# ErlerPhilipp/points2surf

Hardware: NVIDIA H100
Metric: SDF queries/sec at grid_res=256 (higher is better)
Workload: dtype f16 operands / f32 accumulate (wgmma); hi/lo split f16 (fp32-level) for FC tails and guard-band recompute

## Files before the change

points2surf_b200/csrc/net_tc.cu:

```cuda
#include "model.cuh"
#include "tc_ptx.cuh"

namespace p2s {

using namespace ptx;

namespace {

constexpr int kTile = 64;
constexpr int kWG = 2;
constexpr int kThreads = 128 * kWG;
constexpr uint32_t kAct2Bytes = kTile * 128 * 2;
template <bool PRECISE>
struct Cfg {
    static constexpr int kChunks = PRECISE ? 1 : 4;
    static constexpr int kSplit = 8 / kChunks;
    static constexpr uint32_t kChunkBytes = PRECISE ? 65536u : 32768u;
    static constexpr uint32_t kW3Bytes = kChunks * kChunkBytes;
    static constexpr uint32_t kMidScale = PRECISE ? 2u : 1u;
    static constexpr uint32_t kMidBytes = (8192u + 8192u + 16384u) * kMidScale;
    static constexpr uint32_t kPerqBytes = PRECISE ? 16384u : 8192u;
    static constexpr uint32_t kOffMid = kW3Bytes;
    static constexpr uint32_t kWgPerq = kAct2Bytes * kMidScale;
    static constexpr uint32_t kWgWq = kWgPerq + kPerqBytes;
    static constexpr uint32_t kWgBytes = kWgWq + 192 * 4;
    static constexpr uint32_t kOffWg = kOffMid + kMidBytes;
    static constexpr uint32_t kOffBias = kOffWg + kWG * kWgBytes;
    static constexpr uint32_t kSmemBytes = kOffBias + 320 * 4;
};
static_assert(Cfg<false>::kSmemBytes <= 232448 && Cfg<true>::kSmemBytes <= 232448, "shared memory budget");

struct Seg {
    const float* ptr;
    int n;
    int tiles;
    int center;
};

struct PassParams {
    Seg seg[2];
    const float* query;
    const float* R;
    int tiles_per_query;
    int B;
    const float* W0;
    const float* b0;
    int num_mid;
    int mid_N[3];
    const uint8_t* mid_img[3];
    const float* mid_bias[3];
    int perq_layer;
    const uint8_t* perq_img;
    const uint8_t* w3_img;
    float* out;
};

__device__ __forceinline__ uint32_t pack_relu(float a, float b) {
    uint32_t r;
    asm("cvt.rn.relu.satfinite.f16x2.f32 %0, %1, %2;" : "=r"(r) : "f"(b), "f"(a));
    return r;
}
__device__ __forceinline__ void pack_relu_split(float a, float b, uint32_t& hi, uint32_t& lo) {
    hi = pack_relu(a, b);
    const float2 hf = __half22float2(*reinterpret_cast<const __half2*>(&hi));
    lo = pack_half2(fmaxf(a, 0.f) - hf.x, fmaxf(b, 0.f) - hf.y);
}
template <bool PRECISE>
__device__ __forceinline__ void pack_act(float a, float b, uint32_t& hi, uint32_t& lo) {
    if (PRECISE) pack_relu_split(a, b, hi, lo);
    else hi = pack_relu(a, b);
}

template <bool PRECISE, int R>
__device__ __forceinline__ void mid_mma(float (&d)[R], const uint32_t (&a)[4], const uint32_t (&al)[4], uint64_t w, uint64_t w_lo, uint32_t acc) {
    if (R == 32) {
        auto& d32 = reinterpret_cast<float (&)[32]>(d);
        if (PRECISE) { wgmma_rs_n64(d32, al, w, acc); wgmma_rs_n64(d32, a, w_lo, 1); wgmma_rs_n64(d32, a, w, 1); }
        else wgmma_rs_n64(d32, a, w, acc);
    } else {
        auto& d64 = reinterpret_cast<float (&)[64]>(d);
        if (PRECISE) { wgmma_rs_n128(d64, al, w, acc); wgmma_rs_n128(d64, a, w_lo, 1); wgmma_rs_n128(d64, a, w, 1); }
        else wgmma_rs_n128(d64, a, w, acc);
    }
}

template <bool PRECISE>
__global__ void __launch_bounds__(kThreads, 1) pointnet_pass_kernel(const PassParams p) {
    using C = Cfg<PRECISE>;
    constexpr int kL = PRECISE ? 4 : 1;
    extern __shared__ __align__(1024) uint8_t smem[];
    float* s_bias = reinterpret_cast<float*>(smem + C::kOffBias);
    const int tid = threadIdx.x, wg = tid >> 7, t = tid & 127, lane = tid & 31, q4 = lane & 3;
    const int r0 = (t >> 5) * 16 + (lane >> 2);
    const int part = blockIdx.x % C::kSplit;
    const int stream = blockIdx.x / C::kSplit, nstreams = gridDim.x / C::kSplit;
    const int nq = (p.B > stream) ? (p.B - stream + nstreams - 1) / nstreams : 0;
    const int tpq = p.tiles_per_query;
    uint32_t mid_off[3] = {0, 0, 0};
    {
        uint32_t o = 0;
        for (int l = 0; l < p.num_mid; ++l) { mid_off[l] = o; o += (uint32_t)p.mid_N[l] * 128u * C::kMidScale; }
    }

    if (nq > 0) {
        const uint4* src = reinterpret_cast<const uint4*>(p.w3_img + (size_t)part * C::kW3Bytes);
        uint4* dst = reinterpret_cast<uint4*>(smem);
        for (uint32_t i = tid; i < C::kW3Bytes / 16; i += kThreads) dst[i] = src[i];
        for (int l = 0; l < p.num_mid; ++l) {
            if (l == p.perq_layer) continue;
            const uint4* s = reinterpret_cast<const uint4*>(p.mid_img[l]);
            uint4* d = reinterpret_cast<uint4*>(smem + C::kOffMid + mid_off[l]);
            for (uint32_t i = tid; i < (uint32_t)p.mid_N[l] * 8u * C::kMidScale; i += kThreads) d[i] = s[i];
        }
    }
    {
        int off = 0;
        for (int l = 0; l < p.num_mid; ++l) {
            for (int i = tid; i < p.mid_N[l]; i += kThreads) s_bias[off + i] = p.mid_bias[l][i];
            off += p.mid_N[l];
        }
        for (int i = tid; i < 64; i += kThreads) s_bias[256 + i] = p.b0[i];
    }
    fence_proxy_async_smem();
    __syncthreads();

    uint8_t* wsm = smem + C::kOffWg + wg * C::kWgBytes;
    uint8_t* act2 = wsm;
    uint8_t* perq = wsm + C::kWgPerq;
    float* wq = reinterpret_cast<float*>(wsm + C::kWgWq);
    const float* s_b0 = s_bias + 256;
    const uint32_t bar_id = 1 + (uint32_t)wg;
    auto wg_sync = [&]() { asm volatile("bar.sync %0, 128;" ::"r"(bar_id) : "memory"); };
    const uint64_t dsc_act2 = make_smem_desc(smem_u32(act2), 128, 2048);
    const uint64_t dsc_w3 = make_smem_desc(smem_u32(smem), 128, 2048);
    uint64_t dsc_mid[3], dsc_mid_lo[3];
    for (int l = 0; l < 3; ++l) {
        const bool pq = l == p.perq_layer;
        dsc_mid[l] = make_smem_desc(pq ? smem_u32(perq) : smem_u32(smem + C::kOffMid) + mid_off[l], 128, 1024);
        dsc_mid_lo[l] = dsc_mid[l] + (uint64_t)((pq ? 8192u : (uint32_t)p.mid_N[l] * 128u) >> 4);
    }

    for (int qi = wg; qi < nq; qi += kWG) {
        const size_t q = (size_t)stream + (size_t)qi * nstreams;
        wg_sync();
        if (t < 64) {
            const float w0 = p.W0[t * 3 + 0], w1 = p.W0[t * 3 + 1], w2 = p.W0[t * 3 + 2];
            float r[9] = {1.f, 0.f, 0.f, 0.f, 1.f, 0.f, 0.f, 0.f, 1.f};
            if (p.R) {
#pragma unroll
                for (int i = 0; i < 9; ++i) r[i] = p.R[q * 9 + i];
            }
            wq[0 * 64 + t] = w0 * r[0] + w1 * r[3] + w2 * r[6];
            wq[1 * 64 + t] = w0 * r[1] + w1 * r[4] + w2 * r[7];
            wq[2 * 64 + t] = w0 * r[2] + w1 * r[5] + w2 * r[8];
        }
        if (p.perq_layer >= 0) {
            const uint4* s = reinterpret_cast<const uint4*>(p.perq_img + q * C::kPerqBytes);
            uint4* d = reinterpret_cast<uint4*>(perq);
            for (uint32_t i = t; i < C::kPerqBytes / 16; i += 128) d[i] = s[i];
            fence_proxy_async_smem();
        }
        wg_sync();
        float rmax[4 * C::kChunks];
#pragma unroll
        for (int i = 0; i < 4 * C::kChunks; ++i) rmax[i] = -INFINITY;
        for (int tq = 0; tq < tpq; ++tq) {
            const int sgi = tq < p.seg[0].tiles ? 0 : 1;
            const Seg& sg = p.seg[sgi];
            float cx = 0.f, cy = 0.f, cz = 0.f;
            if (sg.center) { cx = p.query[q * 3 + 0]; cy = p.query[q * 3 + 1]; cz = p.query[q * 3 + 2]; }
            float px[2], py[2], pz[2];
#pragma unroll
            for (int h = 0; h < 2; ++h) {
                int local = (tq - (sgi ? p.seg[0].tiles : 0)) * kTile + r0 + 8 * h;
                if (local >= sg.n) local = 0;
                const float* src = sg.ptr + (q * sg.n + local) * 3;
                px[h] = src[0] - cx; py[h] = src[1] - cy; pz[h] = src[2] - cz;
            }
            uint32_t a[4][4], al[4][kL];
#pragma unroll
            for (int kk = 0; kk < 4; ++kk) {
#pragma unroll
                for (int hc = 0; hc < 2; ++hc) {
                    const int ch = kk * 16 + hc * 8 + 2 * q4;
                    const float2 wx = *reinterpret_cast<const float2*>(wq + 0 * 64 + ch);
                    const float2 wy = *reinterpret_cast<const float2*>(wq + 1 * 64 + ch);
                    const float2 wz = *reinterpret_cast<const float2*>(wq + 2 * 64 + ch);
                    const float2 bb = *reinterpret_cast<const float2*>(s_b0 + ch);
#pragma unroll
                    for (int h = 0; h < 2; ++h) {
                        const float v0 = fmaf(wx.x, px[h], fmaf(wy.x, py[h], fmaf(wz.x, pz[h], bb.x)));
                        const float v1 = fmaf(wx.y, px[h], fmaf(wy.y, py[h], fmaf(wz.y, pz[h], bb.y)));
                        pack_act<PRECISE>(v0, v1, a[kk][hc * 2 + h], al[kk][PRECISE ? hc * 2 + h : 0]);
                    }
                }
            }
            int boff = 0;
            for (int l = 0; l < p.num_mid; ++l) {
                const float* bl = s_bias + boff;
                const uint64_t w = dsc_mid[l], w_lo = dsc_mid_lo[l];
                if (l < p.num_mid - 1) {
                    float d[32];
#pragma unroll
                    for (int i = 0; i < 32; ++i) d[i] = 0.f;
                    wgmma_fence();
#pragma unroll
                    for (int ks = 0; ks < 4; ++ks)
                        mid_mma<PRECISE>(d, a[ks], reinterpret_cast<const uint32_t (&)[4]>(al[PRECISE ? ks : 0]), w + (uint64_t)(ks * 16), w_lo + (uint64_t)(ks * 16), ks > 0);
                    wgmma_commit();
                    wgmma_wait<0>();
                    fence_regs(d);
#pragma unroll
                    for (int j = 0; j < 8; ++j) {
                        const float2 bb = *reinterpret_cast<const float2*>(bl + 8 * j + 2 * q4);
                        pack_act<PRECISE>(d[4 * j] + bb.x, d[4 * j + 1] + bb.y, a[j >> 1][(j & 1) * 2], al[j >> 1][PRECISE ? (j & 1) * 2 : 0]);
                        pack_act<PRECISE>(d[4 * j + 2] + bb.x, d[4 * j + 3] + bb.y, a[j >> 1][(j & 1) * 2 + 1], al[j >> 1][PRECISE ? (j & 1) * 2 + 1 : 0]);
                    }
                } else {
                    float d[64];
#pragma unroll
                    for (int i = 0; i < 64; ++i) d[i] = 0.f;
                    wgmma_fence();
#pragma unroll
                    for (int ks = 0; ks < 4; ++ks)
                        mid_mma<PRECISE>(d, a[ks], reinterpret_cast<const uint32_t (&)[4]>(al[PRECISE ? ks : 0]), w + (uint64_t)(ks * 16), w_lo + (uint64_t)(ks * 16), ks > 0);
                    wgmma_commit();
                    wgmma_wait<0>();
                    fence_regs(d);
                    wg_sync();
#pragma unroll
                    for (int j = 0; j < 16; ++j) {
                        const int k = 8 * j + 2 * q4;
                        const float2 bb = *reinterpret_cast<const float2*>(bl + k);
#pragma unroll
                        for (int h = 0; h < 2; ++h) {
                            const int pt = r0 + 8 * h;
                            const uint32_t off = (uint32_t)(pt >> 3) * 2048u + (uint32_t)j * 128u + (uint32_t)(pt & 7) * 16u + (uint32_t)q4 * 4u;
                            uint32_t hi, lo = 0;
                            pack_act<PRECISE>(d[4 * j + 2 * h] + bb.x, d[4 * j + 2 * h + 1] + bb.y, hi, lo);
                            *reinterpret_cast<uint32_t*>(act2 + off) = hi;
                            if (PRECISE) *reinterpret_cast<uint32_t*>(act2 + kAct2Bytes + off) = lo;
                        }
                    }
                    fence_proxy_async_smem();
                    wg_sync();
                }
                boff += p.mid_N[l];
            }
#pragma unroll
            for (int c = 0; c < C::kChunks; ++c) {
                float d0[32], d1[32];
#pragma unroll
                for (int i = 0; i < 32; ++i) { d0[i] = 0.f; d1[i] = 0.f; }
                const uint64_t wa = dsc_w3 + (uint64_t)((uint32_t)c * (C::kChunkBytes >> 4)), wb = wa + (uint64_t)(16384u >> 4);
                wgmma_fence();
#pragma unroll
                for (int ks = 0; ks < 8; ++ks) {
                    const uint64_t x = dsc_act2 + (uint64_t)(ks * 16), o = (uint64_t)(ks * 16);
                    if (PRECISE) {
                        const uint64_t x_lo = x + (uint64_t)(kAct2Bytes >> 4), lo = (uint64_t)(32768u >> 4);
                        wgmma_ss_n64(d0, wa + lo + o, x, ks > 0); wgmma_ss_n64(d0, wa + o, x_lo, 1); wgmma_ss_n64(d0, wa + o, x, 1);
                        wgmma_ss_n64(d1, wb + lo + o, x, ks > 0); wgmma_ss_n64(d1, wb + o, x_lo, 1); wgmma_ss_n64(d1, wb + o, x, 1);
                    } else {
                        wgmma_ss_n64(d0, wa + o, x, ks > 0);
                        wgmma_ss_n64(d1, wb + o, x, ks > 0);
                    }
                }
                wgmma_commit();
                wgmma_wait<0>();
                fence_regs(d0);
                fence_regs(d1);
#pragma unroll
                for (int j = 0; j < 8; ++j) {
                    rmax[4 * c + 0] = fmaxf(rmax[4 * c + 0], fmaxf(d0[4 * j], d0[4 * j + 1]));
                    rmax[4 * c + 1] = fmaxf(rmax[4 * c + 1], fmaxf(d0[4 * j + 2], d0[4 * j + 3]));
                    rmax[4 * c + 2] = fmaxf(rmax[4 * c + 2], fmaxf(d1[4 * j], d1[4 * j + 1]));
                    rmax[4 * c + 3] = fmaxf(rmax[4 * c + 3], fmaxf(d1[4 * j + 2], d1[4 * j + 3]));
                }
            }
        }
#pragma unroll
        for (int i = 0; i < 4 * C::kChunks; ++i) {
            rmax[i] = fmaxf(rmax[i], __shfl_xor_sync(0xffffffffu, rmax[i], 1));
            rmax[i] = fmaxf(rmax[i], __shfl_xor_sync(0xffffffffu, rmax[i], 2));
        }
        if (q4 == 0) {
#pragma unroll
            for (int i = 0; i < 4 * C::kChunks; ++i)
                p.out[q * 1024 + (size_t)((part * C::kChunks + (i >> 2)) * 128 + ((i >> 1) & 1) * 64 + r0 + (i & 1) * 8)] = rmax[i];
        }
    }
}

__global__ void pack_kmajor_kernel(const float* __restrict__ W, int rows, int K, int row0, uint32_t sbo, uint8_t* __restrict__ img, int lo) {
    int e = blockIdx.x * blockDim.x + threadIdx.x;
    if (e >= rows * K) return;
    int r = e / K, k = e % K;
    uint32_t off = (uint32_t)(r >> 3) * sbo + (uint32_t)(k >> 3) * 128u + (uint32_t)(r & 7) * 16u + (uint32_t)(k & 7) * 2u;
    const float w = W[(size_t)(row0 + r) * K + k];
    const __half h = __float2half_rn(w);
    *reinterpret_cast<__half*>(img + off) = lo ? __float2half_rn(w - __half2float(h)) : h;
}

__global__ void pack_perq_kernel(const float* __restrict__ W, int64_t B, uint8_t* __restrict__ img) {
    int64_t e = (int64_t)blockIdx.x * blockDim.x + threadIdx.x;
    if (e >= B * 4096) return;
    int64_t b = e >> 12;
    int r = (int)((e >> 6) & 63), k = (int)(e & 63);
    uint32_t off = (uint32_t)(r >> 3) * 1024u + (uint32_t)(k >> 3) * 128u + (uint32_t)(r & 7) * 16u + (uint32_t)(k & 7) * 2u;
    *reinterpret_cast<__half*>(img + b * 8192 + off) = __float2half_rn(W[e]);
}

__global__ void __launch_bounds__(256) fold_w1_kernel(const float* __restrict__ W1, const float* __restrict__ T, int64_t B, uint8_t* __restrict__ img) {
    __shared__ float sW[64][65];
    __shared__ __align__(16) float sT[64][68];
    const int64_t b = blockIdx.x;
    const int tid = threadIdx.x;
    for (int e = tid; e < 4096; e += 256) {
        const int r = e >> 6, c = e & 63;
        sW[r][c] = W1[e];
        sT[r][c] = T[b * 4096 + e] + (r == c ? 1.0f : 0.0f);
    }
    __syncthreads();
    const int o = tid >> 2, i0 = (tid & 3) * 16;
    float acc[16];
#pragma unroll
    for (int i = 0; i < 16; ++i) acc[i] = 0.f;
    for (int j = 0; j < 64; ++j) {
        const float w = sW[o][j];
#pragma unroll
        for (int i4 = 0; i4 < 4; ++i4) {
            const float4 t4 = *reinterpret_cast<const float4*>(&sT[j][i0 + 4 * i4]);
            acc[4 * i4 + 0] = fmaf(w, t4.x, acc[4 * i4 + 0]);
            acc[4 * i4 + 1] = fmaf(w, t4.y, acc[4 * i4 + 1]);
            acc[4 * i4 + 2] = fmaf(w, t4.z, acc[4 * i4 + 2]);
            acc[4 * i4 + 3] = fmaf(w, t4.w, acc[4 * i4 + 3]);
        }
    }
    uint8_t* dst = img + b * 8192 + (uint32_t)(o >> 3) * 1024u + (uint32_t)(o & 7) * 16u;
#pragma unroll
    for (int h = 0; h < 2; ++h) {
        uint32_t v[4];
#pragma unroll
        for (int e = 0; e < 4; ++e) v[e] = pack_half2(acc[h * 8 + 2 * e], acc[h * 8 + 2 * e + 1]);
        *reinterpret_cast<uint4*>(dst + (uint32_t)(i0 / 8 + h) * 128u) = make_uint4(v[0], v[1], v[2], v[3]);
    }
}

__global__ void fold_fc3_kernel(const float* __restrict__ W1, const float* __restrict__ Wfc3, const float* __restrict__ bfc3,
                                float* __restrict__ G, float* __restrict__ g0) {
    const int oi = blockIdx.x;
    const int o = oi >> 6, i = oi & 63;
    const int k = threadIdx.x;
    float acc = 0.f;
    for (int j = 0; j < 64; ++j) acc = fmaf(W1[o * 64 + j], Wfc3[(size_t)(j * 64 + i) * 256 + k], acc);
    G[(size_t)oi * 256 + k] = acc;
    if (k == 0) {
        float b = W1[o * 64 + i];
        for (int j = 0; j < 64; ++j) b = fmaf(W1[o * 64 + j], bfc3[j * 64 + i], b);
        g0[oi] = b;
    }
}

__global__ void transpose64_kernel(const float* __restrict__ in, float* __restrict__ out, int64_t B) {
    int64_t e = (int64_t)blockIdx.x * blockDim.x + threadIdx.x;
    if (e >= B * 4096) return;
    int64_t b = e >> 12;
    int i = (int)((e >> 6) & 63), j = (int)(e & 63);
    out[e] = in[b * 4096 + j * 64 + i];
}

__global__ void guard_flag_kernel(const float* __restrict__ logits, int64_t B, float band, int32_t* __restrict__ list, int* __restrict__ count, int64_t base, int64_t cap) {
    int64_t i = (int64_t)blockIdx.x * blockDim.x + threadIdx.x;
    if (i >= B) return;
    if (fabsf(logits[i * 2 + 1]) < band) {
        int slot = atomicAdd(count, 1);
        if (slot < cap) list[slot] = (int32_t)(base + i);
    }
}
__global__ void guard_gather_kernel(const float* __restrict__ src, const int32_t* __restrict__ list, int n, int row_floats, float* __restrict__ dst) {
    int64_t e = (int64_t)blockIdx.x * blockDim.x + threadIdx.x;
    if (e >= (int64_t)n * row_floats) return;
    int i = (int)(e / row_floats), j = (int)(e % row_floats);
    dst[e] = src[(int64_t)list[i] * row_floats + j];
}
__global__ void guard_scatter_kernel(const float* __restrict__ src, const int32_t* __restrict__ list, int n, float* __restrict__ logits) {
    int i = blockIdx.x * blockDim.x + threadIdx.x;
    if (i >= n) return;
    logits[(int64_t)list[i] * 2 + 0] = src[i * 2 + 0];
    logits[(int64_t)list[i] * 2 + 1] = src[i * 2 + 1];
}

}

struct TcStack {
    uint8_t* w3_img = nullptr;
    uint8_t* mid_img[3] = {nullptr, nullptr, nullptr};
    uint8_t* w3_img_p = nullptr;
    uint8_t* mid_img_p[3] = {nullptr, nullptr, nullptr};
    const float* mid_bias[3] = {nullptr, nullptr, nullptr};
    int mid_N[3] = {0, 0, 0};
    int num_mid = 0;
    const float* W0 = nullptr;
    const float* b0 = nullptr;
    const float* b3 = nullptr;
};

struct TcFc {
    const Layer* L = nullptr;
    const uint8_t* img = nullptr;
};
struct TcStnFc { TcFc fc1, fc2, fc3; };

struct TcWeights {
    TcStack qstn;
    TcStack stn[2], fin[2];
    TcStnFc qstn_fc, stn_fc[2];
    TcFc head_fc1[2], head_fc2, head_fc3;
    const uint8_t* fold_img[2] = {nullptr, nullptr};
    const float* fold_bias[2] = {nullptr, nullptr};
    bool fc_on_tc = true;
    std::vector<void*> allocs;
    int sm_count = 132;
    bool prof_on = false;
    std::vector<std::pair<cudaEvent_t, cudaEvent_t>> prof_events;
    double prof_flops = 0.0;
    ~TcWeights() {
        for (void* a : allocs) cudaFree(a);
        for (auto& e : prof_events) { cudaEventDestroy(e.first); cudaEventDestroy(e.second); }
    }
};

namespace {

uint8_t* tc_alloc(TcWeights& t, size_t bytes) {
    void* p = nullptr;
    P2S_CUDA(cudaMalloc(&p, bytes));
    P2S_CUDA(cudaMemset(p, 0, bytes));
    t.allocs.push_back(p);
    return (uint8_t*)p;
}

uint8_t* pack_layer(TcWeights& t, const Layer& L, uint32_t sbo, bool split = false) {
    const size_t one = (size_t)L.cout * L.cin * 2;
    uint8_t* img = tc_alloc(t, one * (split ? 2 : 1));
    P2S_LAUNCH(pack_kmajor_kernel, (unsigned)cdiv((int64_t)L.cout * L.cin, 256), 256, 0, 0, L.W, L.cout, L.cin, 0, sbo, img, 0);
    if (split) P2S_LAUNCH(pack_kmajor_kernel, (unsigned)cdiv((int64_t)L.cout * L.cin, 256), 256, 0, 0, L.W, L.cout, L.cin, 0, sbo, img + one, 1);
    return img;
}

uint8_t* pack_w3(TcWeights& t, const Layer& L, bool split = false) {
    P2S_CHECK(L.cout == 1024 && L.cin == 128, "big layer must be 128 -> 1024");
    const size_t chunk = split ? 65536 : 32768;
    uint8_t* img = tc_alloc(t, 8 * chunk);
    for (int c = 0; c < 8; ++c) {
        P2S_LAUNCH(pack_kmajor_kernel, (unsigned)cdiv(128 * 128, 256), 256, 0, 0, L.W, 128, 128, c * 128, 2048u, img + (size_t)c * chunk, 0);
        if (split) P2S_LAUNCH(pack_kmajor_kernel, (unsigned)cdiv(128 * 128, 256), 256, 0, 0, L.W, 128, 128, c * 128, 2048u, img + (size_t)c * chunk + 32768, 1);
    }
    return img;
}

void launch_pass(Model& m, const TcStack& s, const Seg& s0, const Seg& s1, const float* query, const float* R,
                 int64_t B, int perq_layer, const uint8_t* perq_img, float* out, cudaStream_t st, bool precise) {
    PassParams p{};
    p.seg[0] = s0; p.seg[1] = s1;
    p.query = query; p.R = R;
    p.tiles_per_query = s0.tiles + s1.tiles;
    p.B = (int)B;
    p.W0 = s.W0; p.b0 = s.b0;
    p.num_mid = s.num_mid;
    for (int l = 0; l < 3; ++l) { p.mid_N[l] = s.mid_N[l]; p.mid_img[l] = precise ? s.mid_img_p[l] : s.mid_img[l]; p.mid_bias[l] = s.mid_bias[l]; }
    p.perq_layer = perq_layer;
    p.perq_img = perq_img;
    p.w3_img = precise ? s.w3_img_p : s.w3_img;
    p.out = out;
    for (int l = 0; l < s.num_mid; ++l)
        P2S_CHECK(s.mid_N[l] == (l == s.num_mid - 1 ? 128 : 64), "pass kernel: mid layers must be 64 -> 64 ... -> 128");
    TcWeights& t = *m.tc;
    const int split = precise ? Cfg<true>::kSplit : Cfg<false>::kSplit;
    int streams = t.sm_count / split;
    if ((int64_t)streams > B) streams = (int)B;
    const int grid = streams * split;
    cudaEvent_t e0 = nullptr, e1 = nullptr;
    const bool prof = t.prof_on && !precise;
    if (prof) {
        P2S_CUDA(cudaEventCreate(&e0)); P2S_CUDA(cudaEventCreate(&e1));
        P2S_CUDA(cudaEventRecord(e0, st));
    }
    if (precise) P2S_LAUNCH(pointnet_pass_kernel<true>, grid, kThreads, Cfg<true>::kSmemBytes, st, p);
    else P2S_LAUNCH(pointnet_pass_kernel<false>, grid, kThreads, Cfg<false>::kSmemBytes, st, p);
    if (prof) {
        P2S_CUDA(cudaEventRecord(e1, st));
        t.prof_events.emplace_back(e0, e1);
        double mac_pt = 3.0 * 64 + 128.0 * 1024;
        int prev = 64;
        for (int l = 0; l < s.num_mid; ++l) { mac_pt += (double)prev * s.mid_N[l]; prev = s.mid_N[l]; }
        t.prof_flops += 2.0 * mac_pt * (double)(s0.n + s1.n) * (double)B;
    }
}

Seg make_seg(const float* ptr, int n, int center) { return Seg{ptr, n, n > 0 ? (n + kTile - 1) / kTile : 0, center}; }

void run_fc(const TcFc& f, const float* in, int lda, float* out, int ldc, int64_t Bc, bool relu, bool on_tc, cudaStream_t st,
            const float* in_bias = nullptr, bool in_relu = false) {
    const Layer& L = *f.L;
    if (on_tc && f.img) launch_fc_tc(in, lda, f.img, L.b, out, ldc, Bc, L.cout, L.cin, relu, st, 0, in_bias, in_relu);
    else {
        P2S_CHECK(!in_bias, "input bias needs the tensor-core FC kernel");
        launch_gemm_nt(in, 0, lda, L.W, 0, L.b, out, 0, ldc, (int)Bc, L.cout, L.cin, 1, relu, st);
    }
}

void fc_tail(const Layer& b3src, const TcStnFc& s, bool on_tc, const float* gmax_raw, int64_t Bc, float* g, float* f1, float* f2, float* out, cudaStream_t st) {
    if (on_tc && s.fc1.img) run_fc(s.fc1, gmax_raw, 1024, f1, 512, Bc, true, true, st, b3src.b, true);
    else {
        P2S_CUDA(cudaMemcpyAsync(g, gmax_raw, (size_t)Bc * 1024 * 4, cudaMemcpyDeviceToDevice, st));
        launch_bias_act(g, b3src.b, Bc, 1024, true, st);
        run_fc(s.fc1, g, 1024, f1, 512, Bc, true, on_tc, st);
    }
    run_fc(s.fc2, f1, 512, f2, 256, Bc, true, on_tc, st);
    run_fc(s.fc3, f2, 256, out, s.fc3.L->cout, Bc, false, on_tc, st);
}

}

void tc_build(Model& m) {
    P2S_CHECK(m.cfg.net_size == 1024, "tensor-core path needs net_size 1024");
    TcWeights* t = new TcWeights();
    m.tc = t;
    cudaDeviceProp prop;
    P2S_CUDA(cudaGetDeviceProperties(&prop, m.device));
    t->sm_count = prop.multiProcessorCount;
    P2S_CUDA(cudaFuncSetAttribute(pointnet_pass_kernel<false>, cudaFuncAttributeMaxDynamicSharedMemorySize, (int)Cfg<false>::kSmemBytes));
    P2S_CUDA(cudaFuncSetAttribute(pointnet_pass_kernel<true>, cudaFuncAttributeMaxDynamicSharedMemorySize, (int)Cfg<true>::kSmemBytes));
    auto build_stn = [&](TcStack& s, const Stn& stn, const Layer* c0a, const Layer* c0b) {
        if (!c0a) {
            s.W0 = stn.c1.W; s.b0 = stn.c1.b;
            s.num_mid = 1;
            s.mid_img[0] = pack_layer(*t, stn.c2, 1024); s.mid_bias[0] = stn.c2.b; s.mid_N[0] = 128;
            s.mid_img_p[0] = pack_layer(*t, stn.c2, 1024, true);
        } else {
            s.W0 = c0a->W; s.b0 = c0a->b;
            s.num_mid = 3;
            s.mid_img[0] = pack_layer(*t, *c0b, 1024); s.mid_bias[0] = c0b->b; s.mid_N[0] = 64;
            s.mid_img[1] = pack_layer(*t, stn.c1, 1024); s.mid_bias[1] = stn.c1.b; s.mid_N[1] = 64;
            s.mid_img[2] = pack_layer(*t, stn.c2, 1024); s.mid_bias[2] = stn.c2.b; s.mid_N[2] = 128;
            s.mid_img_p[0] = pack_layer(*t, *c0b, 1024, true);
            s.mid_img_p[1] = pack_layer(*t, stn.c1, 1024, true);
            s.mid_img_p[2] = pack_layer(*t, stn.c2, 1024, true);
        }
        s.w3_img_p = pack_w3(*t, stn.c3, true);
        s.w3_img = pack_w3(*t, stn.c3);
        s.b3 = stn.c3.b;
    };
    auto build_fin = [&](TcStack& s, const Feat& f) {
        s.W0 = f.conv0a.W; s.b0 = f.conv0a.b;
        s.num_mid = 3;
        s.mid_img[0] = pack_layer(*t, f.conv0b, 1024); s.mid_bias[0] = f.conv0b.b; s.mid_N[0] = 64;
        s.mid_img[1] = nullptr; s.mid_bias[1] = f.conv1.b; s.mid_N[1] = 64;
        s.mid_img[2] = pack_layer(*t, f.conv2, 1024); s.mid_bias[2] = f.conv2.b; s.mid_N[2] = 128;
        s.mid_img_p[0] = pack_layer(*t, f.conv0b, 1024, true);
        s.mid_img_p[2] = pack_layer(*t, f.conv2, 1024, true);
        s.w3_img_p = pack_w3(*t, f.conv3, true);
        s.w3_img = pack_w3(*t, f.conv3);
        s.b3 = f.conv3.b;
    };
    fc_tc_init();
    {
        const char* e = getenv("P2S_FC_FP32");
        t->fc_on_tc = !(e && e[0] == '1');
    }
    auto mk_fc = [&](const Layer& L) {
        TcFc f;
        f.L = &L;
        f.img = fc_tc_supported(L.cout, L.cin) ? fc_tc_pack(L, t->allocs) : nullptr;
        return f;
    };
    auto mk_stn_fc = [&](const Stn& s) { TcStnFc r; r.fc1 = mk_fc(s.fc1); r.fc2 = mk_fc(s.fc2); r.fc3 = mk_fc(s.fc3); return r; };
    if (m.shared_qstn) t->qstn_fc = mk_stn_fc(m.point_stn);
    else if (m.global.has_qstn) t->qstn_fc = mk_stn_fc(m.global.stn1);
    t->stn_fc[0] = mk_stn_fc(m.local.stn2);
    t->stn_fc[1] = mk_stn_fc(m.global.stn2);
    for (int br = 0; br < 2; ++br) {
        const Feat& f = br ? m.global : m.local;
        P2S_CHECK(f.stn2.fc3.cout == 4096 && f.stn2.fc3.cin == 256 && f.conv1.cout == 64 && f.conv1.cin == 64, "unexpected STN shape");
        float* G = reinterpret_cast<float*>(tc_alloc(*t, (size_t)4096 * 256 * 4));
        float* g0 = reinterpret_cast<float*>(tc_alloc(*t, 4096 * 4));
        P2S_LAUNCH(fold_fc3_kernel, 4096, 256, 0, 0, f.conv1.W, f.stn2.fc3.W, f.stn2.fc3.b, G, g0);
        t->fold_img[br] = fc_tc_pack_raw(G, 4096, 256, t->allocs);
        t->fold_bias[br] = g0;
    }
    t->head_fc1[0] = mk_fc(m.fc1_local);
    t->head_fc1[1] = mk_fc(m.fc1_global);
    t->head_fc2 = mk_fc(m.fc2);
    t->head_fc3 = mk_fc(m.fc3);
    if (m.shared_qstn) build_stn(t->qstn, m.point_stn, nullptr, nullptr);
    else if (m.global.has_qstn) build_stn(t->qstn, m.global.stn1, nullptr, nullptr);
    build_stn(t->stn[0], m.local.stn2, &m.local.conv0a, &m.local.conv0b);
    build_stn(t->stn[1], m.global.stn2, &m.global.conv0a, &m.global.conv0b);
    build_fin(t->fin[0], m.local);
    build_fin(t->fin[1], m.global);
    P2S_CUDA(cudaDeviceSynchronize());
}

void tc_destroy(Model& m) {
    delete m.tc;
    m.tc = nullptr;
}

void tc_profile_reset(Model& m, bool on) {
    TcWeights& t = *m.tc;
    for (auto& e : t.prof_events) { cudaEventDestroy(e.first); cudaEventDestroy(e.second); }
    t.prof_events.clear();
    t.prof_flops = 0.0;
    t.prof_on = on;
}

void tc_profile_get(Model& m, double* ms, int64_t* launches, double* flops) {
    TcWeights& t = *m.tc;
    double total = 0.0;
    for (auto& e : t.prof_events) {
        P2S_CUDA(cudaEventSynchronize(e.second));
        float x = 0.f;
        P2S_CUDA(cudaEventElapsedTime(&x, e.first, e.second));
        total += x;
    }
    *ms = total;
    *launches = (int64_t)t.prof_events.size();
    *flops = t.prof_flops;
}

static void forward_tc_core(Model& m, const float* patch, const float* sub, const float* query, int64_t B,
                            float* logits, cudaStream_t st, bool precise) {
    TcWeights& t = *m.tc;
    const int P = m.cfg.points_per_patch, S = m.cfg.sub_sample_size;
    const int64_t Bc_max = 8192;
    const size_t per_q = 1024 * 4 + 512 + 256 + 4 + 9 + 4096 * 2 + 1024 + 256 + 128 + 4096  + 16 +
                         1024 + 512 + 256 ;
    float* base = m.ws_net.as<float>(per_q * (size_t)Bc_max + 1024);
    float* pcur = base;
    auto take = [&](size_t n) { float* r = pcur; pcur += (n * (size_t)Bc_max + 63) / 64 * 64; return r; };
    float* gmax = take(1024); float* g = take(1024); float* f1 = take(512); float* f2 = take(256);
    float* q4 = take(4); float* R = take(9); float* T = take(4096); float* Tt = take(4096);
    float* fmax_l = take(1024); float* fmax_g = take(1024); float* cat = take(1024); float* h3 = take(256); float* h4 = take(128);
    uint8_t* perq = reinterpret_cast<uint8_t*>(take(4096));
    uint8_t* imgA = reinterpret_cast<uint8_t*>(take(1024)); uint8_t* imgB = reinterpret_cast<uint8_t*>(take(512)); uint8_t* imgC = reinterpret_cast<uint8_t*>(take(256));
    const bool fc_tc = t.fc_on_tc || precise;
    auto img_ok = [](const TcStnFc& f) { return f.fc1.img && f.fc2.img; };
    auto stn_tail_img = [&](const Layer& c3, const TcStnFc& f, const float* gmax_raw, int64_t Bc, float* out_f2) {
        launch_pack_a(gmax_raw, 1024, Bc, 1024, c3.b, true, imgA, st);
        launch_fc_tc_img(imgA, f.fc1.img, f.fc1.L->b, imgB, 0, Bc, 512, 1024, true, st, 3, 16, 0);
        if (out_f2) launch_fc_tc_img(imgB, f.fc2.img, f.fc2.L->b, out_f2, 256, Bc, 256, 512, true, st, 0);
        else launch_fc_tc_img(imgB, f.fc2.img, f.fc2.L->b, imgC, 0, Bc, 256, 512, true, st, 3, 8, 0);
    };

    for (int64_t b0 = 0; b0 < B; b0 += Bc_max) {
        const int64_t Bc = (B - b0 < Bc_max) ? (B - b0) : Bc_max;
        const float* pa = patch + b0 * P * 3;
        const float* su = sub + b0 * S * 3;
        const float* qu = query + b0 * 3;
        const float* Rq = nullptr;
        if (m.shared_qstn) {
            { StageScope ts("net: pass kernels", st); launch_pass(m, t.qstn, make_seg(pa, P, 0), make_seg(su, S, 1), qu, nullptr, Bc, -1, nullptr, gmax, st, precise); }
            { StageScope ts("net: fc tails", st);
              if (fc_tc && img_ok(t.qstn_fc)) {
                  stn_tail_img(m.point_stn.c3, t.qstn_fc, gmax, Bc, f2);
                  run_fc(t.qstn_fc.fc3, f2, 256, q4, 4, Bc, false, false, st);
              } else fc_tail(m.point_stn.c3, t.qstn_fc, fc_tc, gmax, Bc, g, f1, f2, q4, st); }
            launch_quat_to_rot(q4, R, Bc, st);
            Rq = R;
        } else if (m.global.has_qstn) {
            launch_pass(m, t.qstn, make_seg(su, S, 1), make_seg(nullptr, 0, 0), qu, nullptr, Bc, -1, nullptr, gmax, st, precise);
            if (fc_tc && img_ok(t.qstn_fc)) {
                stn_tail_img(m.global.stn1.c3, t.qstn_fc, gmax, Bc, f2);
                run_fc(t.qstn_fc.fc3, f2, 256, q4, 4, Bc, false, false, st);
            } else fc_tail(m.global.stn1.c3, t.qstn_fc, fc_tc, gmax, Bc, g, f1, f2, q4, st);
            launch_quat_to_rot(q4, R, Bc, st);
            Rq = R;
        }
        for (int br = 1; br >= 0; --br) {
            const Feat& f = br ? m.global : m.local;
            const Seg sg = br ? make_seg(su, S, 1) : make_seg(pa, P, 0);
            float* fmax = br ? fmax_g : fmax_l;
            { StageScope ts("net: pass kernels", st); launch_pass(m, t.stn[br], sg, make_seg(nullptr, 0, 0), qu, Rq, Bc, -1, nullptr, gmax, st, precise); }
            if (fc_tc) {
                StageScope ts("net: fc tails", st);
                if (img_ok(t.stn_fc[br])) {
                    stn_tail_img(f.stn2.c3, t.stn_fc[br], gmax, Bc, nullptr);
                    launch_fc_tc_img(imgC, t.fold_img[br], t.fold_bias[br], perq, 0, Bc, 4096, 256, false, st, precise ? 2 : 1);
                } else {
                    run_fc(t.stn_fc[br].fc1, gmax, 1024, f1, 512, Bc, true, true, st, f.stn2.c3.b, true);
                    run_fc(t.stn_fc[br].fc2, f1, 512, f2, 256, Bc, true, true, st);
                    launch_fc_tc(f2, 256, t.fold_img[br], t.fold_bias[br], reinterpret_cast<float*>(perq), 0, Bc, 4096, 256, false, st, precise ? 2 : 1);
                }
            } else {
                { StageScope ts("net: fc tails", st); fc_tail(f.stn2.c3, t.stn_fc[br], false, gmax, Bc, g, f1, f2, T, st); }
                { StageScope ts("net: fold W1*T", st); P2S_LAUNCH(fold_w1_kernel, (unsigned)Bc, 256, 0, st, f.conv1.W, T, Bc, perq); }
            }
            (void)Tt;
            { StageScope ts("net: pass kernels", st); launch_pass(m, t.fin[br], sg, make_seg(nullptr, 0, 0), qu, Rq, Bc, 1, perq, fmax, st, precise); }
        }
        const bool fuse_b3 = fc_tc && !m.debug_aux && t.head_fc1[0].img && t.head_fc1[1].img;
        if (!fuse_b3) {
            launch_bias_act(fmax_l, m.local.conv3.b, Bc, 1024, false, st);
            launch_bias_act(fmax_g, m.global.conv3.b, Bc, 1024, false, st);
        }
        debug_aux_copy(m, b0, Bc, Rq, fmax_l, fmax_g, st);
        StageScope ts_head("net: fc tails", st);
        if (fuse_b3 && t.head_fc2.img && t.head_fc3.img) {
            uint8_t* imgCat = reinterpret_cast<uint8_t*>(cat);
            launch_pack_a(fmax_l, 1024, Bc, 1024, m.local.conv3.b, false, imgA, st);
            launch_fc_tc_img(imgA, t.head_fc1[0].img, m.fc1_local.b, imgCat, 0, Bc, 512, 1024, true, st, 3, 32, 0);
            launch_pack_a(fmax_g, 1024, Bc, 1024, m.global.conv3.b, false, imgA, st);
            launch_fc_tc_img(imgA, t.head_fc1[1].img, m.fc1_global.b, imgCat, 0, Bc, 512, 1024, true, st, 3, 32, 16);
            launch_fc_tc_img(imgCat, t.head_fc2.img, m.fc2.b, imgC, 0, Bc, 256, 1024, true, st, 3, 8, 0);
            launch_fc_tc_img(imgC, t.head_fc3.img, m.fc3.b, h4, 128, Bc, 128, 256, true, st, 0);
        } else {
            run_fc(t.head_fc1[0], fmax_l, 1024, cat, 1024, Bc, true, fc_tc, st, fuse_b3 ? m.local.conv3.b : nullptr, false);
            run_fc(t.head_fc1[1], fmax_g, 1024, cat + 512, 1024, Bc, true, fc_tc, st, fuse_b3 ? m.global.conv3.b : nullptr, false);
            run_fc(t.head_fc2, cat, 1024, h3, 256, Bc, true, fc_tc, st);
            run_fc(t.head_fc3, h3, 256, h4, 128, Bc, true, fc_tc, st);
        }
        launch_gemm_nt(h4, 0, 128, m.fc4.W, 0, m.fc4.b, logits + b0 * 2, 0, 2, (int)Bc, 2, 128, 1, false, st);
    }
}

void forward_guard(Model& m, const float* patch, const float* sub, const float* query, int64_t B, float* logits, cudaStream_t st) {
    static int use_fp32 = -1;
    if (use_fp32 < 0) { const char* e = getenv("P2S_GUARD_FP32"); use_fp32 = (e && e[0] == '1') ? 1 : 0; }
    if (use_fp32) forward_fp32(m, patch, sub, query, B, logits, st);
    else forward_tc_core(m, patch, sub, query, B, logits, st, true);
}

void forward_tc(Model& m, const float* patch, const float* sub, const float* query, int64_t B,
                float* logits, cudaStream_t st) {
    const int P = m.cfg.points_per_patch, S = m.cfg.sub_sample_size;
    forward_tc_core(m, patch, sub, query, B, logits, st, false);

    if (m.guard_band > 0.f && m.guard_list) {
        P2S_LAUNCH(guard_flag_kernel, (unsigned)cdiv(B, 256), 256, 0, st, logits, B, m.guard_band, m.guard_list, m.guard_list_count, m.guard_base, m.guard_list_cap);
    } else if (m.guard_band > 0.f) {
        StageScope ts_guard("net: guard-band fp32 recompute", st);
        int32_t* list = m.ws_guard.as<int32_t>((size_t)B + 64);
        int* count = reinterpret_cast<int*>(list + B);
        P2S_CUDA(cudaMemsetAsync(count, 0, sizeof(int), st));
        P2S_LAUNCH(guard_flag_kernel, (unsigned)cdiv(B, 256), 256, 0, st, logits, B, m.guard_band, list, count, (int64_t)0, B);
        int n = 0;
        P2S_CUDA(cudaMemcpyAsync(&n, count, sizeof(int), cudaMemcpyDeviceToHost, st));
        P2S_CUDA(cudaStreamSynchronize(st));
        m.last_guard_count += n;
        if (n > 0) {
            const size_t rowp = (size_t)P * 3, rows = (size_t)S * 3;
            float* gbuf = m.ws_misc.as<float>((size_t)n * (rowp + rows + 3 + 2) + 64);
            float* gp = gbuf; float* gs = gp + (size_t)n * rowp; float* gq = gs + (size_t)n * rows; float* gl = gq + ((size_t)n * 3 + 3) / 4 * 4;
            P2S_LAUNCH(guard_gather_kernel, (unsigned)cdiv((int64_t)n * rowp, 256), 256, 0, st, patch, list, n, (int)rowp, gp);
            P2S_LAUNCH(guard_gather_kernel, (unsigned)cdiv((int64_t)n * rows, 256), 256, 0, st, sub, list, n, (int)rows, gs);
            P2S_LAUNCH(guard_gather_kernel, (unsigned)cdiv((int64_t)n * 3, 256), 256, 0, st, query, list, n, 3, gq);
            forward_guard(m, gp, gs, gq, n, gl, st);
            P2S_LAUNCH(guard_scatter_kernel, (unsigned)cdiv(n, 256), 256, 0, st, gl, list, n, logits);
        }
    }
}

}
```

Before: 321,000.

## Swap final-layer GEMM operands so activations stay in registers with pipelined wgmma

The last FC layer now takes the mid-layer activations directly from registers as the wgmma A operand, with the transposed role of points and channels, instead of writing them to a shared-memory staging buffer and re-reading them via descriptors. This removes the act2 smem round trip and its two barriers per tile. The output-channel blocks are double-buffered so one wgmma group runs while the previous block's max-reduction executes. The max over points now needs cross-warp shuffles and a small smem reduction buffer with one barrier at the end of each query, and per-layer descriptors are recomputed inside the loop.

```diff
diff --git a/points2surf_b200/csrc/net_tc.cu b/points2surf_b200/csrc/net_tc.cu
--- a/points2surf_b200/csrc/net_tc.cu
+++ b/points2surf_b200/csrc/net_tc.cu
@@ -10,7 +10,6 @@
 constexpr int kTile = 64;
 constexpr int kWG = 2;
 constexpr int kThreads = 128 * kWG;
-constexpr uint32_t kAct2Bytes = kTile * 128 * 2;
 template <bool PRECISE>
 struct Cfg {
     static constexpr int kChunks = PRECISE ? 1 : 4;
@@ -20,10 +19,11 @@
     static constexpr uint32_t kMidScale = PRECISE ? 2u : 1u;
     static constexpr uint32_t kMidBytes = (8192u + 8192u + 16384u) * kMidScale;
     static constexpr uint32_t kPerqBytes = PRECISE ? 16384u : 8192u;
+    static constexpr int kBlocks = kChunks * 2;
     static constexpr uint32_t kOffMid = kW3Bytes;
-    static constexpr uint32_t kWgPerq = kAct2Bytes * kMidScale;
-    static constexpr uint32_t kWgWq = kWgPerq + kPerqBytes;
-    static constexpr uint32_t kWgBytes = kWgWq + 192 * 4;
+    static constexpr uint32_t kWgWq = kPerqBytes;
+    static constexpr uint32_t kWgRed = kWgWq + 192 * 4;
+    static constexpr uint32_t kWgBytes = kWgRed + 4 * kBlocks * 64 * 4;
     static constexpr uint32_t kOffWg = kOffMid + kMidBytes;
     static constexpr uint32_t kOffBias = kOffWg + kWG * kWgBytes;
     static constexpr uint32_t kSmemBytes = kOffBias + 320 * 4;
@@ -96,20 +96,16 @@
     const int stream = blockIdx.x / C::kSplit, nstreams = gridDim.x / C::kSplit;
     const int nq = (p.B > stream) ? (p.B - stream + nstreams - 1) / nstreams : 0;
     const int tpq = p.tiles_per_query;
-    uint32_t mid_off[3] = {0, 0, 0};
-    {
-        uint32_t o = 0;
-        for (int l = 0; l < p.num_mid; ++l) { mid_off[l] = o; o += (uint32_t)p.mid_N[l] * 128u * C::kMidScale; }
-    }
 
     if (nq > 0) {
         const uint4* src = reinterpret_cast<const uint4*>(p.w3_img + (size_t)part * C::kW3Bytes);
         uint4* dst = reinterpret_cast<uint4*>(smem);
         for (uint32_t i = tid; i < C::kW3Bytes / 16; i += kThreads) dst[i] = src[i];
-        for (int l = 0; l < p.num_mid; ++l) {
+        uint32_t moff = 0;
+        for (int l = 0; l < p.num_mid; moff += (uint32_t)p.mid_N[l] * 128u * C::kMidScale, ++l) {
             if (l == p.perq_layer) continue;
             const uint4* s = reinterpret_cast<const uint4*>(p.mid_img[l]);
-            uint4* d = reinterpret_cast<uint4*>(smem + C::kOffMid + mid_off[l]);
+            uint4* d = reinterpret_cast<uint4*>(smem + C::kOffMid + moff);
             for (uint32_t i = tid; i < (uint32_t)p.mid_N[l] * 8u * C::kMidScale; i += kThreads) d[i] = s[i];
         }
     }
@@ -125,20 +121,14 @@
     __syncthreads();
 
     uint8_t* wsm = smem + C::kOffWg + wg * C::kWgBytes;
-    uint8_t* act2 = wsm;
-    uint8_t* perq = wsm + C::kWgPerq;
+    uint8_t* perq = wsm;
     float* wq = reinterpret_cast<float*>(wsm + C::kWgWq);
+    float* red = reinterpret_cast<float*>(wsm + C::kWgRed);
     const float* s_b0 = s_bias + 256;
     const uint32_t bar_id = 1 + (uint32_t)wg;
     auto wg_sync = [&]() { asm volatile("bar.sync %0, 128;" ::"r"(bar_id) : "memory"); };
-    const uint64_t dsc_act2 = make_smem_desc(smem_u32(act2), 128, 2048);
     const uint64_t dsc_w3 = make_smem_desc(smem_u32(smem), 128, 2048);
-    uint64_t dsc_mid[3], dsc_mid_lo[3];
-    for (int l = 0; l < 3; ++l) {
-        const bool pq = l == p.perq_layer;
-        dsc_mid[l] = make_smem_desc(pq ? smem_u32(perq) : smem_u32(smem + C::kOffMid) + mid_off[l], 128, 1024);
-        dsc_mid_lo[l] = dsc_mid[l] + (uint64_t)((pq ? 8192u : (uint32_t)p.mid_N[l] * 128u) >> 4);
-    }
+    const int hb = (lane >> 2) & 1;
 
     for (int qi = wg; qi < nq; qi += kWG) {
         const size_t q = (size_t)stream + (size_t)qi * nstreams;
@@ -161,9 +151,9 @@
             fence_proxy_async_smem();
         }
         wg_sync();
-        float rmax[4 * C::kChunks];
-#pragma unroll
-        for (int i = 0; i < 4 * C::kChunks; ++i) rmax[i] = -INFINITY;
+        float rmax[8 * C::kBlocks];
+#pragma unroll
+        for (int i = 0; i < 8 * C::kBlocks; ++i) rmax[i] = -INFINITY;
         for (int tq = 0; tq < tpq; ++tq) {
             const int sgi = tq < p.seg[0].tiles ? 0 : 1;
             const Seg& sg = p.seg[sgi];
@@ -195,10 +185,14 @@
                     }
                 }
             }
+            uint32_t x[8][4], xl[8][kL];
             int boff = 0;
+            uint32_t moff = 0;
             for (int l = 0; l < p.num_mid; ++l) {
                 const float* bl = s_bias + boff;
-                const uint64_t w = dsc_mid[l], w_lo = dsc_mid_lo[l];
+                const bool pq = l == p.perq_layer;
+                const uint64_t w = make_smem_desc(pq ? smem_u32(perq) : smem_u32(smem + C::kOffMid) + moff, 128, 1024);
+                const uint64_t w_lo = w + (uint64_t)((pq ? 8192u : (uint32_t)p.mid_N[l] * 128u) >> 4);
                 if (l < p.num_mid - 1) {
                     float d[32];
 #pragma unroll
@@ -227,67 +221,70 @@
                     wgmma_commit();
                     wgmma_wait<0>();
                     fence_regs(d);
-                    wg_sync();
 #pragma unroll
                     for (int j = 0; j < 16; ++j) {
-                        const int k = 8 * j + 2 * q4;
-                        const float2 bb = *reinterpret_cast<const float2*>(bl + k);
-#pragma unroll
-                        for (int h = 0; h < 2; ++h) {
-                            const int pt = r0 + 8 * h;
-                            const uint32_t off = (uint32_t)(pt >> 3) * 2048u + (uint32_t)j * 128u + (uint32_t)(pt & 7) * 16u + (uint32_t)q4 * 4u;
-                            uint32_t hi, lo = 0;
-                            pack_act<PRECISE>(d[4 * j + 2 * h] + bb.x, d[4 * j + 2 * h + 1] + bb.y, hi, lo);
-                            *reinterpret_cast<uint32_t*>(act2 + off) = hi;
-                            if (PRECISE) *reinterpret_cast<uint32_t*>(act2 + kAct2Bytes + off) = lo;
+                        const float2 bb = *reinterpret_cast<const float2*>(bl + 8 * j + 2 * q4);
+                        pack_act<PRECISE>(d[4 * j] + bb.x, d[4 * j + 1] + bb.y, x[j >> 1][(j & 1) * 2], xl[j >> 1][PRECISE ? (j & 1) * 2 : 0]);
+                        pack_act<PRECISE>(d[4 * j + 2] + bb.x, d[4 * j + 3] + bb.y, x[j >> 1][(j & 1) * 2 + 1], xl[j >> 1][PRECISE ? (j & 1) * 2 + 1 : 0]);
+                    }
+                }
+                boff += p.mid_N[l];
+                moff += (uint32_t)p.mid_N[l] * 128u * C::kMidScale;
+            }
+            float acc[2][32];
+#pragma unroll
+            for (int b = 0; b <= C::kBlocks; ++b) {
+                if (b < C::kBlocks) {
+                    float (&d)[32] = acc[b & 1];
+                    const uint64_t wb = dsc_w3 + (uint64_t)(((uint32_t)(b >> 1) * C::kChunkBytes + (uint32_t)(b & 1) * 16384u) >> 4);
+                    wgmma_fence();
+#pragma unroll
+                    for (int ks = 0; ks < 8; ++ks) {
+                        const uint64_t w = wb + (uint64_t)(ks * 16);
+                        if (PRECISE) {
+                            wgmma_rs_n64(d, x[ks], w + (uint64_t)(32768u >> 4), ks > 0);
+                            wgmma_rs_n64(d, reinterpret_cast<const uint32_t (&)[4]>(xl[PRECISE ? ks : 0]), w, 1);
+                            wgmma_rs_n64(d, x[ks], w, 1);
+                        } else {
+                            wgmma_rs_n64(d, x[ks], w, ks > 0);
                         }
                     }
-                    fence_proxy_async_smem();
-                    wg_sync();
+                    wgmma_commit();
                 }
-                boff += p.mid_N[l];
-            }
-#pragma unroll
-            for (int c = 0; c < C::kChunks; ++c) {
-                float d0[32], d1[32];
-#pragma unroll
-                for (int i = 0; i < 32; ++i) { d0[i] = 0.f; d1[i] = 0.f; }
-                const uint64_t wa = dsc_w3 + (uint64_t)((uint32_t)c * (C::kChunkBytes >> 4)), wb = wa + (uint64_t)(16384u >> 4);
-                wgmma_fence();
-#pragma unroll
-                for (int ks = 0; ks < 8; ++ks) {
-                    const uint64_t x = dsc_act2 + (uint64_t)(ks * 16), o = (uint64_t)(ks * 16);
-                    if (PRECISE) {
-                        const uint64_t x_lo = x + (uint64_t)(kAct2Bytes >> 4), lo = (uint64_t)(32768u >> 4);
-                        wgmma_ss_n64(d0, wa + lo + o, x, ks > 0); wgmma_ss_n64(d0, wa + o, x_lo, 1); wgmma_ss_n64(d0, wa + o, x, 1);
-                        wgmma_ss_n64(d1, wb + lo + o, x, ks > 0); wgmma_ss_n64(d1, wb + o, x_lo, 1); wgmma_ss_n64(d1, wb + o, x, 1);
-                    } else {
-                        wgmma_ss_n64(d0, wa + o, x, ks > 0);
-                        wgmma_ss_n64(d1, wb + o, x, ks > 0);
+                if (b > 0) {
+                    if (b < C::kBlocks) wgmma_wait<1>();
+                    else wgmma_wait<0>();
+                    float (&d)[32] = acc[(b - 1) & 1];
+                    fence_regs(d);
+                    float* rm = rmax + 8 * (b - 1);
+#pragma unroll
+                    for (int i = 0; i < 4; ++i) {
+#pragma unroll
+                        for (int e = 0; e < 2; ++e) {
+                            const float v0 = fmaxf(d[8 * i + e], d[8 * i + 2 + e]);
+                            const float v1 = fmaxf(d[8 * i + 4 + e], d[8 * i + 6 + e]);
+                            const float other = __shfl_xor_sync(0xffffffffu, hb ? v0 : v1, 4);
+                            rm[2 * i + e] = fmaxf(rm[2 * i + e], fmaxf(hb ? v1 : v0, other));
+                        }
                     }
                 }
-                wgmma_commit();
-                wgmma_wait<0>();
-                fence_regs(d0);
-                fence_regs(d1);
-#pragma unroll
-                for (int j = 0; j < 8; ++j) {
-                    rmax[4 * c + 0] = fmaxf(rmax[4 * c + 0], fmaxf(d0[4 * j], d0[4 * j + 1]));
-                    rmax[4 * c + 1] = fmaxf(rmax[4 * c + 1], fmaxf(d0[4 * j + 2], d0[4 * j + 3]));
-                    rmax[4 * c + 2] = fmaxf(rmax[4 * c + 2], fmaxf(d1[4 * j], d1[4 * j + 1]));
-                    rmax[4 * c + 3] = fmaxf(rmax[4 * c + 3], fmaxf(d1[4 * j + 2], d1[4 * j + 3]));
-                }
             }
         }
 #pragma unroll
-        for (int i = 0; i < 4 * C::kChunks; ++i) {
-            rmax[i] = fmaxf(rmax[i], __shfl_xor_sync(0xffffffffu, rmax[i], 1));
-            rmax[i] = fmaxf(rmax[i], __shfl_xor_sync(0xffffffffu, rmax[i], 2));
-        }
-        if (q4 == 0) {
-#pragma unroll
-            for (int i = 0; i < 4 * C::kChunks; ++i)
-                p.out[q * 1024 + (size_t)((part * C::kChunks + (i >> 2)) * 128 + ((i >> 1) & 1) * 64 + r0 + (i & 1) * 8)] = rmax[i];
+        for (int i = 0; i < 8 * C::kBlocks; ++i) {
+            rmax[i] = fmaxf(rmax[i], __shfl_xor_sync(0xffffffffu, rmax[i], 8));
+            rmax[i] = fmaxf(rmax[i], __shfl_xor_sync(0xffffffffu, rmax[i], 16));
+        }
+        if (lane < 8) {
+            float* rw = red + (t >> 5) * (C::kBlocks * 64);
+#pragma unroll
+            for (int i = 0; i < 8 * C::kBlocks; ++i)
+                rw[(i >> 3) * 64 + 8 * (2 * ((i >> 1) & 3) + hb) + 2 * q4 + (i & 1)] = rmax[i];
+        }
+        wg_sync();
+        for (int c = t; c < C::kBlocks * 64; c += 128) {
+            const float m = fmaxf(fmaxf(red[c], red[C::kBlocks * 64 + c]), fmaxf(red[2 * C::kBlocks * 64 + c], red[3 * C::kBlocks * 64 + c]));
+            p.out[q * 1024 + (size_t)(part * C::kChunks * 128 + c)] = m;
         }
     }
 }
```

Result: faster. 329,600 (median of 6 runs) (+2.7%).
